# MIT-SPARK/Hydra-GNN

Measured on AMD Instinct MI355X. Metric: scene-graphs/sec (fwd+bwd) MP3D hetero batch, higher is better.
Workload: dtype f32

## Files before the change

### hydra-gnn_amd/csrc/aggregate.hip

```cpp
#include <type_traits>

#include "tail_fns.h"

namespace hmp {

KT_DEFINE(agg)
KT_BLOCKS_DEFINE(agg)

__device__ __forceinline__ int cdiv_dev(int a, int b) { return (a + b - 1) / b; }

__device__ __forceinline__ __amdgpu_buffer_rsrc_t buf_rsrc(const void* base, unsigned bytes) {
  return __builtin_amdgcn_make_buffer_rsrc(const_cast<void*>(base), 0, bytes, 0x00020000);
}

template <int VEC>
struct Acc;
template <>
struct Acc<4> {
  float4 v;
  __device__ __forceinline__ void zero() { v = make_float4(0.f, 0.f, 0.f, 0.f); }
  __device__ __forceinline__ void load(const float* p) { v = *reinterpret_cast<const float4*>(p); }
  __device__ __forceinline__ void store(float* p) const { *reinterpret_cast<float4*>(p) = v; }
  __device__ __forceinline__ void add(const Acc& o) { v.x += o.v.x; v.y += o.v.y; v.z += o.v.z; v.w += o.v.w; }
  __device__ __forceinline__ void add_div(const Acc& o, float d) {
// ... 519 lines not shown
    if (oi >= S.n_out) break;
    const TAggOut& O = S.out[oi];
    Acc<VEC> acc[NV];
#pragma unroll
    for (int q = 0; q < NV; ++q) acc[q].zero();
    gather_sum<GS, NV, VEC, GB>(acc, O.g, O.ldg, O.t_col, rb[oi], re[oi], c0, O.F, MeanW{O.rowptr, O.degf, a.mean});
#pragma unroll
    for (int q = 0; q < NV; ++q) {
      const int c = c0 + q * GS * VEC;
      if (c < O.F) put(acc[q], O.coff, c);
    }
  }
  }
  if (S.groot) {
#pragma unroll
    for (int q = 0; q < NV; ++q) {
      const int c = c0 + q * GS * VEC;
      if (c < S.Froot) {
        Acc<VEC> v;
        v.zero();
        if (live) load_z<GB>(v, S.groot, (int64_t)row * S.ldgr + c);
        put(v, S.roff, c);
      }
    }
  }
}

template <int GS, int NV, bool GB = false, bool DZB = false>
__global__ __launch_bounds__(256) void agg_bwd_kernel(const TAggArgs a) {
  if ((int)blockIdx.x == a.total_blocks) {
    finalize_loss(a.fin_row_lv, a.fin_rows, a.fin_out2, a.fin_state);
    return;
  }
  int si = 0;
  while (si + 1 < a.n && (int)blockIdx.x >= a.bstart[si + 1]) ++si;
  karg_warm<10>((int)offsetof(TAggArgs, s) + si * (int)sizeof(TAggSrc), (int)sizeof(TAggSrc));
  const TAggSrc& S = a.s[si];
  const int rpb = (S.tile_rows == 8 && 256 / GS > 8) ? 8 : 256 / GS;
  int local = blockIdx.x - S.block_start;
  if (a.xcd) local = (local & 7) * ((cdiv_dev(S.n_rows, rpb) + 7) >> 3) + (local >> 3);
  if ((int)threadIdx.x / GS >= rpb) return;
  int row = local * rpb + threadIdx.x / GS;
  if (GS == 64) row = __builtin_amdgcn_readfirstlane(row);
  if (row >= S.n_rows) return;
  agg_bwd_row<GS, NV, GB>(a, S, row, true, (int)(threadIdx.x % GS) * 4,
                          [&](Acc<4> v, int seg, int c) { store_z<DZB>(v, S.dz, (int64_t)row * S.lddz + seg + c); });
}

template <int GS>
__device__ __forceinline__ void agg_bwd_dx_tile(const TAggArgs& a, const TAggSrc& S, int row0, int row_end, float* Hs) {
  constexpr int TM = 16, LDH = 17, VEC = 4;
  constexpr int RPP = 256 / GS;
  constexpr int NP = TM / RPP;
  const int tid = threadIdx.x & 255;
  const int c0 = (tid % GS) * VEC;
  const int lane = threadIdx.x & 63, w = tid >> 6;
  const int nn = lane & 15, kq = lane >> 4;
  const int K = S.ncols;
  KT(8);
  constexpr int WB = 48;
#pragma unroll
  for (int p = 0; p < NP; ++p) {
    const int m = p * RPP + tid / GS;
    const int row = row0 + m;
    const bool live = row < row_end;
    agg_bwd_row<GS, 1, false>(a, S, row, live, c0, [&](Acc<VEC> v, int seg, int c) {
      if (live) v.store(S.dz + (int64_t)row * S.lddz + seg + c);
#pragma unroll
      for (int i = 0; i < 4; ++i) Hs[(seg + c + i) * LDH + m] = v.at(i);
    });
  }
  __syncthreads();
  if (S.xw == nullptr) return;
  KT(9);
  const int n_ct = (S.xN + 15) >> 4;
  for (int ct = w; ct < n_ct; ct += 4) {
    const int col = ct * 16 + nn;
    const float* wp = S.xw + min(col, S.xN - 1) + (int64_t)kq * S.xldw;
    const float* hp = Hs + kq * LDH + nn;
    f32x4 acc = {0.f, 0.f, 0.f, 0.f};
    float hv[4] = {0.f, 0.f, 0.f, 0.f};
    if (S.xh) {
#pragma unroll
      for (int r = 0; r < 4; ++r)
        hv[r] = S.xh[(int64_t)min(row0 + kq * 4 + r, row_end - 1) * S.xldh + min(col, S.xN - 1)];
    }
    for (int kb = 0; kb < K; kb += 4 * WB) {
      float bv[WB];
#pragma unroll
      for (int u = 0; u < WB; ++u) bv[u] = wp[(int64_t)min(kb + 4 * u, K - 4) * S.xldw];
#pragma unroll
      for (int u = 0; u < WB; ++u)
        if (kb + 4 * u < K) acc = __builtin_amdgcn_mfma_f32_16x16x4f32(hp[(kb + 4 * u) * LDH], bv[u], acc, 0, 0, 0);
    }
    if (col < S.xN) {
#pragma unroll
      for (int r = 0; r < 4; ++r) {
        const int row = row0 + kq * 4 + r;
        if (row >= row_end) continue;
        float v = acc[r];
        if (S.xh) {
          const float h = hv[r];
          const bool keep = !S.xdrop_on || (__float_as_uint(h) != 0x80000000u);
          float f = S.xscale;
          if (!keep) f = 0.f;
          else if (S.xact == HMP_ACT_RELU) f = h > 0.f ? S.xscale : 0.f;
          else if (S.xact == HMP_ACT_ELU) f = h > 0.f ? S.xscale : (h + S.xscale);
          v *= f;
        }
        S.xg[(int64_t)row * S.xldg + col] = v;
      }
    }
  }
  KT(10);
}

template <int GS>
__global__ __launch_bounds__(256) void agg_bwd_dx_kernel(const TAggArgs a) {
  extern __shared__ float Hs[];
  if ((int)blockIdx.x == a.total_blocks) {
    finalize_loss(a.fin_row_lv, a.fin_rows, a.fin_out2, a.fin_state);
    return;
  }
  KT_SPAN_BEGIN(48);
  int si = 0;
  while (si + 1 < a.n && (int)blockIdx.x >= a.bstart[si + 1]) ++si;
  karg_warm<10>((int)offsetof(TAggArgs, s) + si * (int)sizeof(TAggSrc), (int)sizeof(TAggSrc));
  const TAggSrc& S = a.s[si];
  const int row0 = ((int)blockIdx.x - S.block_start) * S.tile_rows;
  agg_bwd_dx_tile<GS>(a, S, row0, min(row0 + S.tile_rows, S.n_rows), Hs);
  KT_SPAN_END(48, si);
}

constexpr int WIN_THREADS = 1024;
constexpr int WIN_WAVES = WIN_THREADS / 64;
constexpr int WIN_ROW_BYTES = 512;
constexpr int WR = 64;
constexpr int WM = 64;
constexpr int WRING = 256;
constexpr int WG = WR / WIN_WAVES;
constexpr int WIDCAP = 3072;
constexpr int WRP = WR + 1;
constexpr int WIN_LDS_RING = (WRING + 1) * WIN_ROW_BYTES;
constexpr int WIN_LDS_IDS = 2 * WIDCAP * 4;
constexpr int WIN_LDS_RP = 3 * AGG_MAX_IN * WRP * 4;
constexpr int WIN_LDS_DEG = WRING * 4;
constexpr int WIN_LDS_FWD = WIN_LDS_RING + WIN_LDS_IDS + WIN_LDS_RP;
constexpr int WIN_LDS_BWD = WIN_LDS_FWD + WIN_LDS_DEG;
static_assert(WIN_LDS_BWD <= 160 * 1024, "LDS budget");
constexpr unsigned WIN_SKIP_OFF = 0xFFFFF000u;
typedef unsigned int u32x2 __attribute__((ext_vector_type(2)));

static_assert(AGG_MAX_IN == 6, "sel_q is written for 6 entries");
struct WinFwd {
  AggDst d;
  int mean;
  int n_chunks, chunks_per_block;
  int dbg;
};
struct WinBwd {
  TAggSrc s;
  int mean;
  int n_chunks, chunks_per_block;
};

// ... 642 lines not shown
    if (a.s[i].groot) Fmax = a.s[i].Froot > Fmax ? a.s[i].Froot : Fmax;
  }
  return Fmax;
}

int agg_bwd_launch(TAggArgs& a, hipStream_t st) {
  const int vec = 4;
  int Fmax = tagg_fmax(a);
  if (a.n == 0 || Fmax == 0) {
    if (!a.fin_row_lv) return HMP_OK;
    Fmax = 4;
  }
  int gs, nv;
  pick_shape(Fmax, vec, gs, nv);
  int64_t rows_total = 0;
  for (int i = 0; i < a.n; ++i) rows_total += a.s[i].n_rows;
  a.xcd = (rows_total >= AGG_XCD_ROWS && agg_xcd_enabled()) ? 1 : 0;
  for (int i = 0; i < a.n; ++i)
    if (a.xcd || a.gb16 || rows_total > 16 * AGG_SMALL_TILES) a.s[i].tile_rows = 0;
  int blocks = agg_layout_rows(a, gs);
  if (blocks == 0 && !a.fin_row_lv) return HMP_OK;
  if (a.gb16) {
    HMP_CHECK_ARG(gs == 64 && nv == 1, "agg_bwd: bf16 gradient rows need row widths in (128, 256], got %d", Fmax);
    if (agg_win_enabled()) {
      bool any;
      HMP_TRY(agg_win_peel(a, st, &any));
      if (any) {
        blocks = agg_layout_rows(a, gs);
        if (blocks == 0 && !a.fin_row_lv) return HMP_OK;
      }
    }
    const int grid = blocks + (a.fin_row_lv ? 1 : 0);
    sync_bstart(a);
    if (a.dzb16) hipLaunchKernelGGL((agg_bwd_kernel<64, 1, true, true>), dim3(grid), dim3(256), 0, st, a);
    else hipLaunchKernelGGL((agg_bwd_kernel<64, 1, true, false>), dim3(grid), dim3(256), 0, st, a);
    HMP_LAUNCH_CHECK();
    return HMP_OK;
  }
  HMP_CHECK_ARG(!a.dzb16, "agg_bwd: a bf16 dz needs bf16 gradient rows (the one-wavefront-per-row kernel)");
  const int grid = blocks + (a.fin_row_lv ? 1 : 0);
  sync_bstart(a);
#define LAUNCH_BWD(GS_, NV_) hipLaunchKernelGGL((agg_bwd_kernel<GS_, NV_>), dim3(grid), dim3(256), 0, st, a)
  HMP_DISPATCH_GS_NV(gs, nv, LAUNCH_BWD)
#undef LAUNCH_BWD
  HMP_LAUNCH_CHECK();
  return HMP_OK;
}

int agg_bwd_dx_launch(TAggArgs& a, hipStream_t st) {
  int Fmax = tagg_fmax(a), kmax = 0;
  for (int i = 0; i < a.n; ++i) {
    kmax = a.s[i].ncols > kmax ? a.s[i].ncols : kmax;
    HMP_CHECK_ARG((a.s[i].ncols & 3) == 0, "agg_bwd_dx: ncols must be padded to 4");
  }
  if (a.n == 0 || Fmax == 0) {
    if (!a.fin_row_lv) return HMP_OK;
    Fmax = 4;
  }
  HMP_CHECK_ARG(Fmax <= 256 && kmax <= 896, "agg_bwd_dx: segment width %d / stacked width %d not supported", Fmax, kmax);
  const int blocks = agg_layout_tiles(a);
  if (blocks == 0 && !a.fin_row_lv) return HMP_OK;
  const int grid = blocks + (a.fin_row_lv ? 1 : 0);
  const size_t smem = (size_t)kmax * 17 * sizeof(float);
  sync_bstart(a);
  switch (agg_tile_gs(Fmax)) {
    case 16: hipLaunchKernelGGL((agg_bwd_dx_kernel<16>), dim3(grid), dim3(256), smem, st, a); break;
    case 32: hipLaunchKernelGGL((agg_bwd_dx_kernel<32>), dim3(grid), dim3(256), smem, st, a); break;
    default: hipLaunchKernelGGL((agg_bwd_dx_kernel<64>), dim3(grid), dim3(256), smem, st, a); break;
  }
  HMP_LAUNCH_CHECK();
  return HMP_OK;
}

template <bool FWD>
static int segment_mean_dispatch(const float* in, int ldi, int F, const hmp_plan& plan, float* out, int ldo, hipStream_t st) {
  const bool vec_ok = ((ldi & 3) == 0) && ((ldo & 3) == 0) && ((reinterpret_cast<uintptr_t>(in) & 15) == 0) &&
                      ((reinterpret_cast<uintptr_t>(out) & 15) == 0) && ((F & 3) == 0);
  const int vec = vec_ok ? 4 : 1;
  const int Fmax = F;
  const int n_rows = FWD ? plan.n_dst : plan.n_src;
  if (n_rows == 0 || F == 0) return HMP_OK;
  int gs, nv;
  pick_shape(F, vec, gs, nv);
  const int blocks = cdiv(n_rows, 256 / gs);
#define LAUNCH_SM(GS_, NV_)                                                                                                   \
  do {                                                                                                                        \
    if (FWD) {                                                                                                                \
      if (vec_ok) hipLaunchKernelGGL((segment_mean_fwd_kernel<GS_, NV_, 4>), dim3(blocks), dim3(256), 0, st, in, ldi, F, plan.d_rowptr, plan.d_col, n_rows, out, ldo); \
      else hipLaunchKernelGGL((segment_mean_fwd_kernel<GS_, NV_, 1>), dim3(blocks), dim3(256), 0, st, in, ldi, F, plan.d_rowptr, plan.d_col, n_rows, out, ldo); \
    } else {                                                                                                                  \
      if (vec_ok) hipLaunchKernelGGL((segment_mean_bwd_kernel<GS_, NV_, 4>), dim3(blocks), dim3(256), 0, st, in, ldi, F, plan.d_t_rowptr, plan.d_t_col, plan.d_rowptr, n_rows, out, ldo); \
      else hipLaunchKernelGGL((segment_mean_bwd_kernel<GS_, NV_, 1>), dim3(blocks), dim3(256), 0, st, in, ldi, F, plan.d_t_rowptr, plan.d_t_col, plan.d_rowptr, n_rows, out, ldo); \
    }                                                                                                                         \
  } while (0)
  HMP_DISPATCH_GS_NV(gs, nv, LAUNCH_SM)
#undef LAUNCH_SM
  HMP_LAUNCH_CHECK();
  return HMP_OK;
}

}

extern "C" int hmp_segment_mean_fwd(const float* d_x, int32_t ldx, int32_t F, hmp_plan plan, float* d_out, int32_t ldo, void* stream) {
  using namespace hmp;
  HMP_CHECK_ARG(d_x && d_out && plan.d_rowptr, "hmp_segment_mean_fwd: null pointer");
  HMP_CHECK_ARG(F >= 0 && ldx >= F && ldo >= F, "hmp_segment_mean_fwd: bad widths");
  HMP_CHECK_ARG(plan.n_edges == 0 || plan.d_col, "hmp_segment_mean_fwd: null col");
  const int panel = ((ldx & 3) == 0 && (ldo & 3) == 0 && (F & 3) == 0) ? 1024 : 256;
  for (int c = 0; c < F; c += panel) {
    const int w = (F - c) < panel ? (F - c) : panel;
    HMP_TRY((segment_mean_dispatch<true>(d_x + c, ldx, w, plan, d_out + c, ldo, (hipStream_t)stream)));
  }
  return HMP_OK;
}

extern "C" int hmp_segment_mean_bwd(const float* d_gout, int32_t ldg, int32_t F, hmp_plan plan, float* d_gx, int32_t ldgx, void* stream) {
// ... 12 lines not shown
```

### hydra-gnn_amd/csrc/device_fns.h

```cpp
#pragma once
#include "kernels.h"

namespace hmp {

__device__ __forceinline__ int find_seg(const int64_t* __restrict__ off, int B, int64_t g) {
  int lo = 0, hi = B - 1;
  while (lo < hi) {
    const int mid = (lo + hi + 1) >> 1;
    if (off[mid] <= g) lo = mid; else hi = mid - 1;
  }
  return lo;
}


__device__ __forceinline__ void pack_item(const PackSeg& S, int item, const float* __restrict__ params, float* __restrict__ packed) {
  const int chunks = (S.ld_dst + 63) >> 6;
  const int r = item / chunks;
  if (r >= S.rows_pad) return;
  float* dst = packed + S.dst + (int64_t)r * S.ld_dst;
  const int c = (item % chunks) * 64 + (threadIdx.x & 63);
  if (c >= S.ld_dst) return;
  float v = 0.f;
  if (S.kind == PACK_SUM) {
    if (r < S.rows && c < S.cols)
      for (int q = 0; q < S.nsrc; ++q) v += params[S.src[q] + (int64_t)r * S.ld_src + c];
  } else if (S.kind == PACK_HEADS) {
    const int h = r / S.Cp, cc = r % S.Cp;
    if (h < S.H && cc < S.C && c < S.cols) v = params[S.src[0] + (int64_t)(h * S.C + cc) * S.ld_src + c];
  } else if (S.kind == PACK_ATTDOT) {
    if (r < S.H && c < S.cols) {
      const float* av = params + S.att + r * S.C;
      const float* wv = params + S.src[0] + (int64_t)(r * S.C) * S.ld_src + c;
      for (int cc = 0; cc < S.C; cc += 8) {
        float a8[8], w8[8];
#pragma unroll
        for (int u = 0; u < 8; ++u) {
          const int ci = min(cc + u, S.C - 1);
          a8[u] = av[ci];
          w8[u] = wv[(int64_t)ci * S.ld_src];
        }
#pragma unroll
        for (int u = 0; u < 8; ++u)
          if (cc + u < S.C) v += a8[u] * w8[u];
      }
    }
  } else {
    if (r < S.rows && c < S.H) {
      const float* av = params + S.att + c * S.C;
      const float* wv = params + S.src[0] + (int64_t)(c * S.C) * S.ld_src + r;
      for (int cc = 0; cc < S.C; cc += 8) {
        float a8[8], w8[8];
#pragma unroll
        for (int u = 0; u < 8; ++u) {
          const int ci = min(cc + u, S.C - 1);
          a8[u] = av[ci];
          w8[u] = wv[(int64_t)ci * S.ld_src];
        }
#pragma unroll
        for (int u = 0; u < 8; ++u)
          if (cc + u < S.C) v += a8[u] * w8[u];
      }
    }
  }
  dst[c] = v;
}

__device__ __forceinline__ void pack_block(const PackSeg* __restrict__ segs, const SegBlocks& sb, const float* __restrict__ params,
                                           float* __restrict__ packed, int* step_ctr, int* step_mirror, int blk) {
  if (step_ctr && blk == 0 && threadIdx.x == 0) {
    const int t = *step_ctr + 1;
    *step_ctr = t;
    if (step_mirror) *step_mirror = t;
  }
  int si = 0;
  while (si + 1 < sb.n && blk >= sb.start[si + 1]) ++si;
  const PackSeg S = segs[si];
  pack_item(S, (blk - sb.start[si]) * 4 + (int)(threadIdx.x >> 6), params, packed);
}

}
```

### hydra-gnn_amd/csrc/kernels.h

```cpp
#pragma once
#include "common.h"

namespace hmp {

enum { EPI_NONE = 0, EPI_ACTMASK = 1 };

struct GemmProblem {
  const float* A;
  const float* B;
  float* C;
  const float* H;
  int c_bf16;
  int a_bf16;
  int b_bf16;
  int h_bf16;
  const float* A2;
  int lda2, a_split;
  int64_t slab_stride;
  int M, N, K;
  int lda, ldb, ldc, ldh;
  int trans_a;
  int trans_b;
  int n_real;
  int aug_ones;
// ... 209 lines not shown
  int ldzr, roff;
  const float* bias;
  int n_in;
  int act;
  int drop_on;
  DropCfg drop;
  int block_start;
  const float* pw;
  float* pz;
  int pldw, pldz, pncols, pK;
  const int64_t* ce_labels;
  int64_t ce_ignored;
  int ce_classes, ce_ldg;
  float* ce_grad;
  float* ce_row_lv;
  const uint8_t* ce_mask;
  int ce_tail;
  int win_in;
  int tile_rows;
  AggIn in[AGG_MAX_IN];
};
struct AggArgs {
  int n;
  int total_blocks;
  int mean;
  int xcd;
  int zb16;
  int hb16;
  NetState* state;
  int bstart[HMP_MAX_NODE_TYPES];
  AggDst d[HMP_MAX_NODE_TYPES];
};
int agg_fwd_launch(AggArgs& a, hipStream_t st);
int agg_proj_fwd_launch(AggArgs& a, hipStream_t st);

struct TAggOut {
  const int* t_rowptr;
  const int* t_col;
  const int* rowptr;
  const float* degf;
  const float* g;
  int ldg, coff, F;
  int same_type;
  int n_dst;
};
struct TAggSrc {
  int n_rows;
  float* dz;
  int lddz, ncols;
  const float* groot;
  int ldgr, roff, Froot;
  int n_out;
  int block_start;
  const float* xw;
  float* xg;
  const float* xh;
  int xldw, xN, xldg, xldh, xact, xdrop_on;
  float xscale;
  int win_out;
  int tile_rows;
  TAggOut out[AGG_MAX_IN];
};
struct TAggArgs {
  int n;
  int total_blocks;
  int mean;
  int xcd;
  int gb16;
  int dzb16;
  const float* fin_row_lv;
  int fin_rows;
  float* fin_out2;
  NetState* fin_state;
  int bstart[HMP_MAX_NODE_TYPES];
  TAggSrc s[HMP_MAX_NODE_TYPES];
};
int agg_bwd_launch(TAggArgs& a, hipStream_t st);
int agg_bwd_dx_launch(TAggArgs& a, hipStream_t st);

int seg_mean_rows_launch(const void* x, int ldx, int x_bf16, int F, const int* rowptr, const int* col, int n_rows, float* m, int ldm,
                         hipStream_t st);
int seg_mean_rows_t_launch(const float* dm, int lddm, int F, const int* t_rowptr, const int* t_col, const float* degf, int n_rows,
                           const void* h, int ldh, int h_bf16, int act, int drop_on, float dscale, void* g, int ldg, int g_bf16, hipStream_t st);

enum { PACK_SUM = 0, PACK_HEADS = 1, PACK_ATTDOT = 2, PACK_ATTDOT_T = 3 };
struct PackSeg {
  int64_t dst;
  int rows, rows_pad, cols, ld_dst;
  int ld_src;
  int nsrc;
  int kind, H, C, Cp;
  int64_t att;
  int64_t src[AGG_MAX_IN];
};
constexpr int SEG_MAX = 400;
struct SegBlocks {
  int n;
  int start[SEG_MAX + 1];
};
int pack_launch(const PackSeg* d_segs, const SegBlocks& sb, const float* d_params, float* d_packed, int* step_ctr, int* step_mirror,
                hipStream_t st);

enum { GT_COPY = 0, GT_ATT_OUTER = 1, GT_ATT_DOT = 2, GT_ATT_OUTER_T = 3, GT_ATT_DOT_T = 4 };
struct GradTerm {
  int kind;
  int slab_id;
  int64_t src;
  int ld;
  int C, Cp;
  int inner;
  int64_t att, w;
  int ldw;
  float scale;
};
struct GradSeg {
  int64_t dst;
  int rows, cols;
  int n_terms;
  GradTerm t[3];
};
constexpr int SLAB_IDS_PER_LAYER = 2 * HMP_MAX_NODE_TYPES + HMP_MAX_CONVS;
constexpr int GRAD_MAX_SLAB_IDS = HMP_MAX_LAYERS * SLAB_IDS_PER_LAYER;
constexpr int HEAD_SLAB_ID = GRAD_MAX_SLAB_IDS;
struct GradReduceDyn {
  unsigned char n_slabs[GRAD_MAX_SLAB_IDS + 1];
  int slab_stride[GRAD_MAX_SLAB_IDS + 1];
};

constexpr int GAT_HMAX = 8;
constexpr int GAT_MAX_EDIM = 4;
constexpr int GAT_CMAX = 512;
constexpr int GAT_WIDE_HMAX = 4;
inline bool gat_shape_ok(int heads, int channels) {
  return heads >= 1 && heads <= GAT_HMAX && channels >= 1 && channels <= GAT_CMAX && (channels <= 256 || heads <= GAT_WIDE_HMAX);
}

struct GatInS {
  int et, src_t;
  const int *rowptr, *col, *eid, *t_rowptr, *t_col, *t_pos;
  const float* z;
  int ldz, hoff;
  const float* za;
  int ldza, asoff;
  const float* zd;
  int ldzd, adoff;
  const float* vedge;
  int edim;
// ... 153 lines not shown
```

### hydra-gnn_amd/csrc/net.hip

```cpp
#include <cstdlib>
#include <vector>

#include "plan_small.h"

using namespace hmp;

namespace {

struct ConvLayout {
  int coff;
  int asoff, adoff;
  int H, C, Cp;
  int64_t vedge_off;
  int64_t vslab_off;
  bool wd_is_src;
  float *smax, *sden, *alpha_drop, *dlogit, *dlogit_orig;
  bool agg_first;
  int aoff, ld_m;
  int64_t wc_off, cslab_off;
  float *mrows, *dmrows;
};

struct LayerLayout {
  int kind;
  int n_live;
  int live[HMP_MAX_CONVS];
  ConvLayout conv[HMP_MAX_CONVS];
  int n_in[HMP_MAX_NODE_TYPES];
  bool reads[HMP_MAX_NODE_TYPES];
  int aggf_of_src[HMP_MAX_NODE_TYPES];
  int ncols[HMP_MAX_NODE_TYPES];
  int roff[HMP_MAX_NODE_TYPES];
  int64_t wp_off[HMP_MAX_NODE_TYPES];
  int ldw[HMP_MAX_NODE_TYPES];
  int64_t bias_off[HMP_MAX_NODE_TYPES];
  int64_t slab_off[HMP_MAX_NODE_TYPES];
  int lddw[HMP_MAX_NODE_TYPES];
  int64_t bslab_off[HMP_MAX_NODE_TYPES];
  GatLayerS* d_gat;
  GatLayerS h_gat;
};

constexpr int MAX_SLABS = 192;
static_assert(MAX_SLABS >= GEMM_TALL_SLABS, "the slab buffer must hold what the tall weight-gradient kernel may write");
constexpr int TN_DIRECT_SLABS = 16;

struct ProfRec {
  int cls;
  hipEvent_t a, b;
};

}

struct EnvSwitches {
  bool plan_sliced = true;
  bool front = true;
  bool z16 = true;
  bool h16 = true;
  bool rootcopy = false;
  bool tn_direct = true;
  bool bf16_all = false;
};

struct StepCall {
  int training = 0;
  uint64_t seed = 0;
  uint32_t rng_step = 0;
  int* d_step = nullptr;
  const int64_t* ce_labels = nullptr;
  const hmp_head_targets* tgt = nullptr;
  int64_t ce_ignored = 0;
  AdamFuse adam = {};
  bool fin_loss = false;
  int fin_rows = 0;
  bool aux_g_ready = false;
  int head_blocks = 0;
  bool ce_done = false;
  bool tail_done[2] = {false, false};
  bool adam_done = false;
};

struct hmp_net {
  hmp_net_spec spec;
  EnvSwitches env;
  int T, ET, L;
  int dim[HMP_MAX_LAYERS + 1][HMP_MAX_NODE_TYPES];
  int ld[HMP_MAX_LAYERS + 1][HMP_MAX_NODE_TYPES];
// ... 159 lines not shown
      Y.reads[C.src] = Y.reads[C.dst] = true;
      if (Y.kind == HMP_CONV_SAGE) {
        HMP_CHECK_ARG(C.w0 >= 0 && C.b0 >= 0 && C.w1 >= 0, "net: SAGE conv needs lin_l.weight, lin_l.bias, lin_r.weight");
        if (aggf) {
          HMP_CHECK_ARG(Y.aggf_of_src[C.src] < 0, "net: layer %d has two aggregate-first convs from node type %d (at most one)", l, C.src);
          Y.aggf_of_src[C.src] = c;
          Q.agg_first = true;
          Q.ld_m = fpad(n->dim[l][C.src]);
          n->any_agg_first = true;
        } else {
          Q.coff = Y.ncols[C.src];
          Y.ncols[C.src] += fpad(C.f_out);
        }
      } else {
        HMP_CHECK_ARG(C.w0 >= 0 && C.a0 >= 0 && C.a1 >= 0 && C.b0 >= 0, "net: GAT conv needs lin_src, att_src, att_dst, bias");
        HMP_CHECK_ARG(C.edge_dim == 0 || (C.w2 >= 0 && C.a2 >= 0), "net: GAT_edge conv needs lin_edge, att_edge");
        Q.H = C.heads; Q.C = C.f_out; Q.Cp = fpad(C.f_out);
        Q.wd_is_src = (C.src == C.dst) || (C.w1 == C.w0) || (C.w1 < 0);
        HMP_CHECK_ARG(Q.wd_is_src ? (n->dim[l][C.src] == n->dim[l][C.dst]) : true, "net: shared lin with different widths");
        Q.coff = Y.ncols[C.src];
        Y.ncols[C.src] += Q.H * Q.Cp;
        Q.asoff = Y.ncols[C.src];
        Y.ncols[C.src] += fpad(Q.H);
        n->any_gat = true;
      }
    }
    HMP_CHECK_ARG(Y.n_live > 0, "net: layer %d has no live conv", l);
    if (Y.kind == HMP_CONV_SAGE) {
      for (int i = 0; i < Y.n_live; ++i) {
        const int c = Y.live[i];
        const hmp_conv_spec& C = Ls.convs[c];
        if (!Y.conv[c].agg_first) continue;
        Y.conv[c].aoff = Y.ncols[C.dst];
        Y.ncols[C.dst] += fpad(C.f_out);
      }
      for (int t = 0; t < n->T; ++t)
        if (Y.n_in[t] > 0) {
          Y.roff[t] = Y.ncols[t];
          Y.ncols[t] += fpad(Ls.out_dim[t]);
        }
    } else {
      for (int i = 0; i < Y.n_live; ++i) {
        const int c = Y.live[i];
        const hmp_conv_spec& C = Ls.convs[c];
        Y.conv[c].adoff = Y.ncols[C.dst];
        Y.ncols[C.dst] += fpad(C.heads);
      }
    }
    for (int t = 0; t < n->T; ++t) {
      Y.ldw[t] = fpad(n->dim[l][t]);
      Y.lddw[t] = fpad(n->dim[l][t] + 1);
      Y.wp_off[t] = packed;
      packed += (int64_t)Y.ncols[t] * Y.ldw[t];
      Y.bias_off[t] = packed;
      packed += (Y.n_in[t] > 0) ? fpad(Ls.out_dim[t]) : 0;
      Y.slab_off[t] = slabs;
      slabs += (int64_t)MAX_SLABS * Y.ncols[t] * Y.lddw[t];
      Y.bslab_off[t] = slabs;
      if (Y.kind == HMP_CONV_GAT && Y.n_in[t] > 0) slabs += (int64_t)MAX_SLABS * fpad(Ls.out_dim[t]) * 4;
    }
    for (int i = 0; i < Y.n_live; ++i) {
      const int c = Y.live[i];
      if (!Y.conv[c].agg_first) continue;
      const hmp_conv_spec& C = Ls.convs[c];
      Y.conv[c].wc_off = packed;
      packed += (int64_t)fpad(C.f_out) * Y.ldw[C.src];
      Y.conv[c].cslab_off = slabs;
      slabs += (int64_t)MAX_SLABS * fpad(C.f_out) * Y.lddw[C.src];
    }
    if (Y.kind == HMP_CONV_GAT) {
      for (int i = 0; i < Y.n_live; ++i) {
        const int c = Y.live[i];
        if (Ls.convs[c].edge_dim > 0) {
          Y.conv[c].vedge_off = packed;
          packed += GAT_MAX_EDIM * GAT_HMAX;
          Y.conv[c].vslab_off = slabs;
          slabs += (int64_t)MAX_SLABS * GAT_MAX_EDIM * GAT_HMAX;
        }
      }
    }
  }
  for (int l = 0; l < n->L; ++l) {
    const LayerLayout& Y = n->lay[l];
    for (int i = 0; i < Y.n_live; ++i) {
      const hmp_conv_spec& C = S.layers[l].convs[Y.live[i]];
      if (l == n->L - 1)
        HMP_CHECK_ARG(C.dst == S.readout_type || C.dst == S.aux_readout_type,
                      "net: last-layer conv %d is active but does not feed a readout type", Y.live[i]);
      else
        HMP_CHECK_ARG(n->lay[l + 1].reads[C.dst], "net: layer %d conv %d is active but layer %d never reads its output", l, Y.live[i], l + 1);
    }
  }
  n->packed_floats = packed;
  n->slab_floats = slabs;
  n->out_dim = n->dim[n->L][S.readout_type];
  n->out_ld = fpad(n->out_dim);
  HMP_CHECK_ARG(n->out_dim > 0, "net: readout type has no output in the last layer");
  HMP_CHECK_ARG(S.aux_readout_type < 0 || n->dim[n->L][S.aux_readout_type] > 0, "net: second readout type has no output in the last layer");
  return HMP_OK;
}

inline int slab_id_w(int l, int t) { return l * SLAB_IDS_PER_LAYER + t; }
inline int slab_id_b(int l, int t) { return l * SLAB_IDS_PER_LAYER + HMP_MAX_NODE_TYPES + t; }
inline int slab_id_v(int l, int c) { return l * SLAB_IDS_PER_LAYER + 2 * HMP_MAX_NODE_TYPES + c; }

GradTerm term(int kind, int slab_id, int64_t src, int ld, int C, int Cp, int inner = 0, int64_t att = 0, int64_t w = 0, int ldw = 0,
              float scale = 1.f) {
  GradTerm t;
  memset(&t, 0, sizeof(t));
  t.kind = kind; t.slab_id = slab_id; t.src = src; t.ld = ld; t.C = C; t.Cp = Cp; t.inner = inner;
  t.att = att; t.w = w; t.ldw = ldw; t.scale = scale;
  return t;
}

int build_tables(hmp_net* n) {
  const hmp_net_spec& S = n->spec;
  std::vector<PackSeg> ps;
  std::vector<int64_t> prs;
  std::vector<GradSeg> gs;
  std::vector<int64_t> ges;
  int64_t prow = 0, gel = 0;
  auto push_pack = [&](const PackSeg& s) {
    ps.push_back(s); prs.push_back(prow); prow += s.rows_pad;
    if (s.rows_pad > n->max_pack_rows) n->max_pack_rows = s.rows_pad;
  };
  auto push_grad = [&](GradSeg g) {
    gs.push_back(g); ges.push_back(gel); gel += (int64_t)g.rows * g.cols;
    if ((int64_t)g.rows * g.cols > n->max_grad_elems) n->max_grad_elems = (int64_t)g.rows * g.cols;
  };
  for (int l = 0; l < n->L; ++l) {
    const hmp_layer_spec& Ls = S.layers[l];
    const LayerLayout& Y = n->lay[l];
    const float gscale = Ls.group_mean ? 1.f : 1.f;
    (void)gscale;
    for (int i = 0; i < Y.n_live; ++i) {
      const int c = Y.live[i];
      const hmp_conv_spec& C = Ls.convs[c];
      const ConvLayout& Q = Y.conv[c];
      const int fs = n->dim[l][C.src], ft = n->dim[l][C.dst];
      PackSeg s;
      memset(&s, 0, sizeof(s));
      if (Y.kind == HMP_CONV_SAGE) {
        s.kind = PACK_SUM;
        s.dst = Q.agg_first ? Q.wc_off : Y.wp_off[C.src] + (int64_t)Q.coff * Y.ldw[C.src];
        s.rows = C.f_out; s.rows_pad = fpad(C.f_out); s.cols = fs; s.ld_dst = Y.ldw[C.src]; s.ld_src = fs;
        s.nsrc = 1; s.src[0] = C.w0;
        push_pack(s);
        GradSeg g;
        memset(&g, 0, sizeof(g));
        g.dst = C.w0; g.rows = C.f_out; g.cols = fs; g.n_terms = 1;
        if (Q.agg_first) g.t[0] = term(GT_COPY, slab_id_v(l, c), Q.cslab_off, Y.lddw[C.src], C.f_out, C.f_out);
        else g.t[0] = term(GT_COPY, slab_id_w(l, C.src), Y.slab_off[C.src] + (int64_t)Q.coff * Y.lddw[C.src], Y.lddw[C.src], C.f_out, C.f_out);
        push_grad(g);
        continue;
      }
      const int HC = Q.H * Q.C;
      const int64_t wd = Q.wd_is_src ? C.w0 : C.w1;
      s.kind = PACK_HEADS; s.H = Q.H; s.C = Q.C; s.Cp = Q.Cp;
      s.dst = Y.wp_off[C.src] + (int64_t)Q.coff * Y.ldw[C.src];
      s.rows = Q.H * Q.Cp; s.rows_pad = Q.H * Q.Cp; s.cols = fs; s.ld_dst = Y.ldw[C.src]; s.ld_src = fs;
      s.nsrc = 1; s.src[0] = C.w0;
      push_pack(s);
      s.kind = PACK_ATTDOT; s.dst = Y.wp_off[C.src] + (int64_t)Q.asoff * Y.ldw[C.src];
      s.rows = Q.H; s.rows_pad = fpad(Q.H); s.att = C.a0; s.src[0] = C.w0;
      push_pack(s);
      s.dst = Y.wp_off[C.dst] + (int64_t)Q.adoff * Y.ldw[C.dst];
      s.cols = ft; s.ld_dst = Y.ldw[C.dst]; s.ld_src = ft; s.att = C.a1; s.src[0] = wd;
      push_pack(s);
      if (C.edge_dim > 0) {
        s.kind = PACK_ATTDOT_T; s.dst = Q.vedge_off; s.rows = C.edge_dim; s.rows_pad = GAT_MAX_EDIM; s.cols = Q.H;
        s.ld_dst = GAT_HMAX; s.ld_src = C.edge_dim; s.att = C.a2; s.src[0] = C.w2;
        push_pack(s);
      }
      const int64_t S_hs = Y.slab_off[C.src] + (int64_t)Q.coff * Y.lddw[C.src];
      const int64_t S_as = Y.slab_off[C.src] + (int64_t)Q.asoff * Y.lddw[C.src];
      const int64_t S_ad = Y.slab_off[C.dst] + (int64_t)Q.adoff * Y.lddw[C.dst];
      GradSeg g;
      memset(&g, 0, sizeof(g));
      g.dst = C.w0; g.rows = HC; g.cols = fs;
      g.t[g.n_terms++] = term(GT_COPY, slab_id_w(l, C.src), S_hs, Y.lddw[C.src], Q.C, Q.Cp);
      g.t[g.n_terms++] = term(GT_ATT_OUTER, slab_id_w(l, C.src), S_as, Y.lddw[C.src], Q.C, Q.C, 0, C.a0);
      if (Q.wd_is_src) g.t[g.n_terms++] = term(GT_ATT_OUTER, slab_id_w(l, C.dst), S_ad, Y.lddw[C.dst], Q.C, Q.C, 0, C.a1);
      push_grad(g);
      if (!Q.wd_is_src) {
        memset(&g, 0, sizeof(g));
        g.dst = C.w1; g.rows = HC; g.cols = ft; g.n_terms = 1;
        g.t[0] = term(GT_ATT_OUTER, slab_id_w(l, C.dst), S_ad, Y.lddw[C.dst], Q.C, Q.C, 0, C.a1);
        push_grad(g);
      }
      memset(&g, 0, sizeof(g));
      g.dst = C.a0; g.rows = HC; g.cols = 1; g.n_terms = 1;
      g.t[0] = term(GT_ATT_DOT, slab_id_w(l, C.src), S_as, Y.lddw[C.src], Q.C, Q.C, fs, 0, C.w0, fs);
      push_grad(g);
      memset(&g, 0, sizeof(g));
      g.dst = C.a1; g.rows = HC; g.cols = 1; g.n_terms = 1;
      g.t[0] = term(GT_ATT_DOT, slab_id_w(l, C.dst), S_ad, Y.lddw[C.dst], Q.C, Q.C, ft, 0, wd, ft);
      push_grad(g);
      if (C.edge_dim > 0) {
        memset(&g, 0, sizeof(g));
        g.dst = C.w2; g.rows = HC; g.cols = C.edge_dim; g.n_terms = 1;
        g.t[0] = term(GT_ATT_OUTER_T, slab_id_v(l, c), Q.vslab_off, GAT_HMAX, Q.C, Q.C, 0, C.a2);
        push_grad(g);
        memset(&g, 0, sizeof(g));
        g.dst = C.a2; g.rows = HC; g.cols = 1; g.n_terms = 1;
        g.t[0] = term(GT_ATT_DOT_T, slab_id_v(l, c), Q.vslab_off, GAT_HMAX, Q.C, Q.C, C.edge_dim, 0, C.w2, C.edge_dim);
        push_grad(g);
      }
      memset(&g, 0, sizeof(g));
      const int wout = Ls.out_dim[C.dst];
      g.dst = C.b0; g.rows = wout; g.cols = 1; g.n_terms = 1;
      g.t[0] = term(GT_COPY, slab_id_b(l, C.dst), Y.bslab_off[C.dst], 4, wout, wout, 0, 0, 0, 0,
                    Ls.group_mean ? 1.f / (float)Y.n_in[C.dst] : 1.f);
      push_grad(g);
    }
    for (int t = 0; t < n->T; ++t) {
      if (Y.n_in[t] == 0) continue;
      const int fo = Ls.out_dim[t], ft = n->dim[l][t];
      PackSeg s, b;
      memset(&s, 0, sizeof(s));
      memset(&b, 0, sizeof(b));
      s.kind = PACK_SUM; b.kind = PACK_SUM;
      s.dst = Y.wp_off[t] + (int64_t)(Y.roff[t] < 0 ? 0 : Y.roff[t]) * Y.ldw[t];
      s.rows = fo; s.rows_pad = fpad(fo); s.cols = ft; s.ld_dst = Y.ldw[t]; s.ld_src = ft;
      b.dst = Y.bias_off[t];
      b.rows = 1; b.rows_pad = 1; b.cols = fo; b.ld_dst = fpad(fo); b.ld_src = fo;
      for (int i = 0; i < Y.n_live; ++i) {
        const hmp_conv_spec& C = Ls.convs[Y.live[i]];
        if (C.dst != t) continue;
        b.src[b.nsrc++] = C.b0;
        if (Y.kind != HMP_CONV_SAGE) continue;
        s.src[s.nsrc++] = C.w1;
        GradSeg g;
        memset(&g, 0, sizeof(g));
        g.dst = C.w1; g.rows = fo; g.cols = ft; g.n_terms = 1;
        const int64_t root = Y.slab_off[t] + (int64_t)Y.roff[t] * Y.lddw[t];
        g.t[0] = term(GT_COPY, slab_id_w(l, t), root, Y.lddw[t], fo, fo);
        push_grad(g);
        memset(&g, 0, sizeof(g));
        g.dst = C.b0; g.rows = fo; g.cols = 1; g.n_terms = 1;
        g.t[0] = term(GT_COPY, slab_id_w(l, t), root + ft, Y.lddw[t], fo, fo);
        push_grad(g);
      }
      if (Y.kind == HMP_CONV_SAGE) push_pack(s);
      push_pack(b);
    }
  }
  prs.push_back(prow);
  ges.push_back(gel);
  n->n_pack = (int)ps.size(); n->pack_rows = prow;
  n->n_grad = (int)gs.size(); n->grad_elems = gel;
  HMP_CHECK_ARG(ps.size() <= (size_t)SEG_MAX && gs.size() <= (size_t)SEG_MAX, "net: too many parameter segments (%zu / %zu > %d)",
                ps.size(), gs.size(), SEG_MAX);
  n->pack_sb.n = (int)ps.size();
  n->pack_sb.start[0] = 0;
  for (size_t i = 0; i < ps.size(); ++i)
    n->pack_sb.start[i + 1] = n->pack_sb.start[i] + cdiv((int64_t)ps[i].rows_pad * cdiv(ps[i].ld_dst, 64), 4);
  {
    std::vector<int2> pm;
    for (size_t i = 0; i < ps.size(); ++i) {
      const int items = ps[i].rows_pad * cdiv(ps[i].ld_dst, 64);
      for (int it = 0; it < items; it += 16) pm.push_back(make_int2((int)i, it));
    }
    n->n_pack_blocks16 = (int)pm.size();
    if (!pm.empty()) {
      HMP_HIP(hipMalloc(&n->d_pack_map, pm.size() * sizeof(int2)));
      HMP_HIP(hipMemcpy(n->d_pack_map, pm.data(), pm.size() * sizeof(int2), hipMemcpyHostToDevice));
    }
  }
  n->grad_sb.n = (int)gs.size();
  n->grad_sb.start[0] = 0;
  for (size_t i = 0; i < gs.size(); ++i) {
    const bool wave_mode = gs[i].n_terms == 1 && (gs[i].t[0].kind == GT_ATT_DOT || gs[i].t[0].kind == GT_ATT_DOT_T);
    const int64_t el = (int64_t)gs[i].rows * gs[i].cols;
    n->grad_sb.start[i + 1] = n->grad_sb.start[i] + cdiv(el, wave_mode ? 4 : 256);
  }
  HMP_HIP(hipMalloc(&n->d_pack_segs, ps.size() * sizeof(PackSeg)));
  HMP_HIP(hipMalloc(&n->d_grad_segs, gs.size() * sizeof(GradSeg)));
  HMP_HIP(hipMemcpy(n->d_pack_segs, ps.data(), ps.size() * sizeof(PackSeg), hipMemcpyHostToDevice));
  HMP_HIP(hipMemcpy(n->d_grad_segs, gs.data(), gs.size() * sizeof(GradSeg), hipMemcpyHostToDevice));
  for (int l = 0; l < n->L; ++l)
    if (n->lay[l].kind == HMP_CONV_GAT) HMP_HIP(hipMalloc(&n->lay[l].d_gat, sizeof(GatLayerS)));
  return HMP_OK;
}

size_t carve(hmp_net* n, char* base, const int32_t* cn, const int64_t* ce) {
  size_t off = 0;
  n->sadd_floats = 0;
  auto take = [&](size_t bytes) -> char* {
    char* p = base ? base + off : nullptr;
    off += align256(bytes);
    return p;
  };
  const hmp_net_spec& S = n->spec;
  for (int e = 0; e < n->ET; ++e) {
    const int ns = cn[S.edge_src[e]], nd = cn[S.edge_dst[e]];
    hmp_plan& P = n->plan[e];
// ... 670 lines not shown
        n->call.fin_loss = false;
        fin_early = true;
      }
      for (int s = 0; s < n->T; ++s) {
        if (Y.ncols[s] == 0 || b->n_nodes[s] == 0) continue;
        TAggSrc& T = a.s[a.n++];
        T.n_rows = b->n_nodes[s];
        T.dz = n->dZ[l][s]; T.lddz = Y.ncols[s]; T.ncols = Y.ncols[s];
        if (Y.roff[s] >= 0) {
          int ldg;
          T.groot = g_of(s, ldg);
          T.ldgr = ldg; T.roff = Y.roff[s]; T.Froot = fpad(Ls.out_dim[s]);
        }
        for (int i = 0; i < Y.n_live; ++i) {
          const int c = Y.live[i];
          const hmp_conv_spec& C = Ls.convs[c];
          if (Y.conv[c].agg_first) {
            if (C.dst != s || b->n_nodes[C.src] == 0 || b->n_edges[C.edge_type] == 0) continue;
            TAggOut& O = T.out[T.n_out++];
            O.t_rowptr = n->d_iota; O.t_col = n->d_iota; O.rowptr = n->d_iota; O.degf = n->d_ones;
            int ldg;
            O.g = g_of(s, ldg);
            O.ldg = ldg; O.coff = Y.conv[c].aoff; O.F = fpad(C.f_out);
            O.same_type = 0; O.n_dst = b->n_nodes[s];
            continue;
          }
          if (C.src != s) continue;
          TAggOut& O = T.out[T.n_out++];
          const hmp_plan& P = n->plan[C.edge_type];
          O.t_rowptr = P.d_t_rowptr; O.t_col = P.d_t_col; O.rowptr = P.d_rowptr; O.degf = n->degf[C.edge_type];
          int ldg;
          O.g = g_of(C.dst, ldg);
          O.ldg = ldg; O.coff = Y.conv[c].coff; O.F = fpad(C.f_out);
          O.same_type = C.src == C.dst ? 1 : 0;
          O.n_dst = b->n_nodes[C.dst];
          if (n->fuse_now && b->n_edges[C.edge_type] > (int64_t)8 * b->n_nodes[C.src]) T.tile_rows = 8;
        }
      }
      dx_fused = n->fuse_now && l > 0;
      int fmax = 0;
      for (int i = 0; i < a.n && dx_fused; ++i) {
        if (a.s[i].ncols > 896) dx_fused = false;
        for (int o = 0; o < a.s[i].n_out; ++o) fmax = a.s[i].out[o].F > fmax ? a.s[i].out[o].F : fmax;
        if (a.s[i].groot) fmax = a.s[i].Froot > fmax ? a.s[i].Froot : fmax;
      }
      if (fmax > 256) dx_fused = false;
      if (dx_fused) {
        const hmp_layer_spec& Lp = S.layers[l - 1];
        int ai = 0;
        for (int s = 0; s < n->T; ++s) {
          if (Y.ncols[s] == 0 || b->n_nodes[s] == 0) continue;
          TAggSrc& T = a.s[ai++];
          if (!n->G[l][s]) continue;
          T.xw = n->d_packed + Y.wp_off[s]; T.xldw = Y.ldw[s]; T.xN = n->dim[l][s];
          T.xg = n->G[l][s]; T.xldg = n->ld[l][s];
          T.xdrop_on = (n->training && Lp.dropout > 0.f) ? 1 : 0;
          T.xact = Lp.act;
          T.xscale = T.xdrop_on ? 1.f / (1.f - Lp.dropout) : 1.f;
          T.xh = (T.xact != HMP_ACT_NONE || T.xdrop_on) ? n->H[l][s] : nullptr;
          T.xldh = n->ld[l][s];
        }
        HMP_TRY(agg_bwd_dx_launch(a, st));
      } else {
        a.gb16 = g16[l + 1] ? 1 : 0;
        dz16 = a.gb16 && n->compute_bf16 != 0;
        for (int s = 0; s < n->T && dz16; ++s)
          if (Y.ncols[s] > 0 && b->n_nodes[s] > 0 && (Y.ncols[s] % 256) != 0) dz16 = false;
        if (!n->env.z16) dz16 = false;
        a.dzb16 = dz16 ? 1 : 0;
        rootless = dz16;
        for (int i = 0; i < a.n && rootless; ++i)
          if (a.s[i].groot && ((a.s[i].roff & 255) != 0 || a.s[i].Froot != 256 || (a.s[i].ldgr & 3) != 0)) rootless = false;
        if (n->env.rootcopy) rootless = false;
        if (rootless)
          for (int i = 0; i < a.n; ++i) a.s[i].groot = nullptr;
        HMP_TRY(agg_bwd_launch(a, st));
      }
    }
    const bool need_dx = !dx_fused && ((l > 0) || (d_gx != nullptr));
    auto dz_at = [&](int t, int col) -> const float* {
      return dz16 ? reinterpret_cast<const float*>(reinterpret_cast<const uint16_t*>(n->dZ[l][t]) + col) : n->dZ[l][t] + col;
    };
    auto aggf_live = [&](int c) {
      const hmp_conv_spec& C = Ls.convs[c];
      return Y.conv[c].agg_first && b->n_nodes[C.dst] > 0 && b->n_nodes[C.src] > 0 && b->n_edges[C.edge_type] > 0;
    };
    if (need_dx && n->any_agg_first) {
      std::vector<GemmProblem> pp;
      for (int i = 0; i < Y.n_live; ++i) {
        const int c = Y.live[i];
        if (!aggf_live(c)) continue;
        const hmp_conv_spec& C = Ls.convs[c];
        float* want = l > 0 ? n->G[l][C.src] : d_gx[C.src];
        if (!want) continue;
        const ConvLayout& Q = Y.conv[c];
        GemmProblem p;
        memset(&p, 0, sizeof(p));
        p.A = dz_at(C.dst, Q.aoff); p.lda = Y.ncols[C.dst]; p.trans_a = 0; p.a_bf16 = dz16 ? 1 : 0;
        p.B = n->d_packed + Q.wc_off; p.ldb = Y.ldw[C.src]; p.trans_b = 0;
        p.C = Q.dmrows; p.ldc = Q.ld_m;
        p.M = b->n_nodes[C.dst]; p.N = n->dim[l][C.src]; p.K = fpad(C.f_out);
        p.n_real = p.N;
        p.epi = EPI_NONE;
        pp.push_back(p);
      }
      if (!pp.empty()) {
        Scope sp(n, KC_GEMM_BWD, st);
// ... 801 lines not shown
```

Measured before the change: 371,700.

## Use a transposed, swizzled weight image for vectorized loads in the fused dx GEMM

The parameter packer now also writes a transposed copy of each SAGE layer's weights, with padding and a column swizzle, so the fused input-gradient tile can fetch four K values per lane with one float4 load. Before, it issued one strided scalar load per MFMA step. For the GS=16 variant, the first column tile's weights and activations are prefetched before the barrier so their latency overlaps the aggregation phase. The cost is extra packed-parameter memory, extra packing writes every step, a larger padded shared-memory tile, and higher register pressure from the prefetch buffer.

```diff
diff --git a/hydra-gnn_amd/csrc/aggregate.hip b/hydra-gnn_amd/csrc/aggregate.hip
--- a/hydra-gnn_amd/csrc/aggregate.hip
+++ b/hydra-gnn_amd/csrc/aggregate.hip
@@ -595,13 +595,28 @@
   constexpr int TM = 16, LDH = 17, VEC = 4;
   constexpr int RPP = 256 / GS;
   constexpr int NP = TM / RPP;
+  constexpr int WB = 12;
   const int tid = threadIdx.x & 255;
   const int c0 = (tid % GS) * VEC;
   const int lane = threadIdx.x & 63, w = tid >> 6;
   const int nn = lane & 15, kq = lane >> 4;
-  const int K = S.ncols;
+  const int K = S.ncols, K16 = (K + 15) & ~15;
   KT(8);
-  constexpr int WB = 48;
+  constexpr bool EARLY = GS == 16;
+  const int n_ct = S.xwt ? (S.xN + 15) >> 4 : 0;
+  float4 pre[WB];
+  auto fetch_first = [&]() {
+    if (w >= n_ct) return;
+    const float* wrow = S.xwt + (int64_t)min(w * 16 + nn, S.xN - 1) * S.xldt + 4 * kq;
+#pragma unroll
+    for (int i = 0; i < WB; ++i) pre[i] = *reinterpret_cast<const float4*>(wrow + min(16 * i, K16 - 16));
+  };
+  float hv0[4] = {0.f, 0.f, 0.f, 0.f};
+  if (EARLY && S.xh && w < n_ct) {
+#pragma unroll
+    for (int r = 0; r < 4; ++r)
+      hv0[r] = S.xh[(int64_t)min(row0 + kq * 4 + r, row_end - 1) * S.xldh + min(w * 16 + nn, S.xN - 1)];
+  }
 #pragma unroll
   for (int p = 0; p < NP; ++p) {
     const int m = p * RPP + tid / GS;
@@ -613,28 +628,46 @@
       for (int i = 0; i < 4; ++i) Hs[(seg + c + i) * LDH + m] = v.at(i);
     });
   }
+  if constexpr (EARLY) fetch_first();
+  for (int i = tid; i < (K16 - K) * TM; i += 256) Hs[(K + (i >> 4)) * LDH + (i & 15)] = 0.f;
   __syncthreads();
-  if (S.xw == nullptr) return;
+  if (S.xwt == nullptr) return;
   KT(9);
-  const int n_ct = (S.xN + 15) >> 4;
-  for (int ct = w; ct < n_ct; ct += 4) {
+  auto trip = [&](int kb, const float4 (&bv)[WB], f32x4& acc) {
+#pragma unroll
+    for (int i = 0; i < WB; ++i) {
+      const int k = kb + 16 * i;
+      if (k >= K) break;
+      const float* hp = Hs + (k + kq) * LDH + nn;
+      acc = __builtin_amdgcn_mfma_f32_16x16x4f32(hp[0 * LDH], bv[i].x, acc, 0, 0, 0);
+      acc = __builtin_amdgcn_mfma_f32_16x16x4f32(hp[4 * LDH], bv[i].y, acc, 0, 0, 0);
+      acc = __builtin_amdgcn_mfma_f32_16x16x4f32(hp[8 * LDH], bv[i].z, acc, 0, 0, 0);
+      acc = __builtin_amdgcn_mfma_f32_16x16x4f32(hp[12 * LDH], bv[i].w, acc, 0, 0, 0);
+    }
+  };
+  auto tile = [&](int ct, auto first) {
     const int col = ct * 16 + nn;
-    const float* wp = S.xw + min(col, S.xN - 1) + (int64_t)kq * S.xldw;
-    const float* hp = Hs + kq * LDH + nn;
+    const float* wrow = S.xwt + (int64_t)min(col, S.xN - 1) * S.xldt + 4 * kq;
     f32x4 acc = {0.f, 0.f, 0.f, 0.f};
     float hv[4] = {0.f, 0.f, 0.f, 0.f};
-    if (S.xh) {
+    if constexpr (decltype(first)::value) {
+#pragma unroll
+      for (int r = 0; r < 4; ++r) hv[r] = hv0[r];
+    } else if (S.xh) {
 #pragma unroll
       for (int r = 0; r < 4; ++r)
         hv[r] = S.xh[(int64_t)min(row0 + kq * 4 + r, row_end - 1) * S.xldh + min(col, S.xN - 1)];
     }
-    for (int kb = 0; kb < K; kb += 4 * WB) {
-      float bv[WB];
-#pragma unroll
-      for (int u = 0; u < WB; ++u) bv[u] = wp[(int64_t)min(kb + 4 * u, K - 4) * S.xldw];
-#pragma unroll
-      for (int u = 0; u < WB; ++u)
-        if (kb + 4 * u < K) acc = __builtin_amdgcn_mfma_f32_16x16x4f32(hp[(kb + 4 * u) * LDH], bv[u], acc, 0, 0, 0);
+    int kb = 0;
+    if constexpr (decltype(first)::value) {
+      trip(0, pre, acc);
+      kb = 16 * WB;
+    }
+    for (; kb < K; kb += 16 * WB) {
+      float4 bv[WB];
+#pragma unroll
+      for (int i = 0; i < WB; ++i) bv[i] = *reinterpret_cast<const float4*>(wrow + min(kb + 16 * i, K16 - 16));
+      trip(kb, bv, acc);
     }
     if (col < S.xN) {
 #pragma unroll
@@ -654,6 +687,12 @@
         S.xg[(int64_t)row * S.xldg + col] = v;
       }
     }
+  };
+  if constexpr (EARLY) {
+    if (w < n_ct) tile(w, std::true_type());
+    for (int ct = w + 4; ct < n_ct; ct += 4) tile(ct, std::false_type());
+  } else {
+    for (int ct = w; ct < n_ct; ct += 4) tile(ct, std::false_type());
   }
   KT(10);
 }
@@ -1402,6 +1441,8 @@
   for (int i = 0; i < a.n; ++i) {
     kmax = a.s[i].ncols > kmax ? a.s[i].ncols : kmax;
     HMP_CHECK_ARG((a.s[i].ncols & 3) == 0, "agg_bwd_dx: ncols must be padded to 4");
+    HMP_CHECK_ARG(!a.s[i].xwt || (a.s[i].xldt == ((a.s[i].ncols + 15) & ~15) && a.s[i].xN > 0),
+                  "agg_bwd_dx: transposed weights of %d columns with leading dimension %d", a.s[i].ncols, a.s[i].xldt);
   }
   if (a.n == 0 || Fmax == 0) {
     if (!a.fin_row_lv) return HMP_OK;
@@ -1411,7 +1452,7 @@
   const int blocks = agg_layout_tiles(a);
   if (blocks == 0 && !a.fin_row_lv) return HMP_OK;
   const int grid = blocks + (a.fin_row_lv ? 1 : 0);
-  const size_t smem = (size_t)kmax * 17 * sizeof(float);
+  const size_t smem = (size_t)((kmax + 15) & ~15) * 17 * sizeof(float);
   sync_bstart(a);
   switch (agg_tile_gs(Fmax)) {
     case 16: hipLaunchKernelGGL((agg_bwd_dx_kernel<16>), dim3(grid), dim3(256), smem, st, a); break;
diff --git a/hydra-gnn_amd/csrc/device_fns.h b/hydra-gnn_amd/csrc/device_fns.h
--- a/hydra-gnn_amd/csrc/device_fns.h
+++ b/hydra-gnn_amd/csrc/device_fns.h
@@ -13,12 +13,13 @@
 }
 
 
-__device__ __forceinline__ void pack_item(const PackSeg& S, int item, const float* __restrict__ params, float* __restrict__ packed) {
+__host__ __device__ __forceinline__ void pack_lane(const PackSeg& S, int item, int lane, const float* __restrict__ params,
+                                                   float* __restrict__ packed) {
   const int chunks = (S.ld_dst + 63) >> 6;
   const int r = item / chunks;
   if (r >= S.rows_pad) return;
   float* dst = packed + S.dst + (int64_t)r * S.ld_dst;
-  const int c = (item % chunks) * 64 + (threadIdx.x & 63);
+  const int c = (item % chunks) * 64 + lane;
   if (c >= S.ld_dst) return;
   float v = 0.f;
   if (S.kind == PACK_SUM) {
@@ -63,6 +64,15 @@
     }
   }
   dst[c] = v;
+  if (S.ld_dst_t > 0) {
+    float* dt = packed + S.dst_t + (int64_t)c * S.ld_dst_t;
+    dt[wpt_col(S.col_t + r)] = v;
+    for (int p = r; p < S.pad_t; p += S.rows_pad) dt[wpt_col(S.col_t + S.rows_pad + p)] = 0.f;
+  }
+}
+
+__device__ __forceinline__ void pack_item(const PackSeg& S, int item, const float* __restrict__ params, float* __restrict__ packed) {
+  pack_lane(S, item, (int)(threadIdx.x & 63), params, packed);
 }
 
 __device__ __forceinline__ void pack_block(const PackSeg* __restrict__ segs, const SegBlocks& sb, const float* __restrict__ params,
diff --git a/hydra-gnn_amd/csrc/kernels.h b/hydra-gnn_amd/csrc/kernels.h
--- a/hydra-gnn_amd/csrc/kernels.h
+++ b/hydra-gnn_amd/csrc/kernels.h
@@ -285,10 +285,10 @@
   int ldgr, roff, Froot;
   int n_out;
   int block_start;
-  const float* xw;
+  const float* xwt;
   float* xg;
   const float* xh;
-  int xldw, xN, xldg, xldh, xact, xdrop_on;
+  int xldt, xN, xldg, xldh, xact, xdrop_on;
   float xscale;
   int win_out;
   int tile_rows;
@@ -325,7 +325,10 @@
   int kind, H, C, Cp;
   int64_t att;
   int64_t src[AGG_MAX_IN];
-};
+  int64_t dst_t;
+  int ld_dst_t, col_t, pad_t;
+};
+__host__ __device__ inline int wpt_col(int k) { return (k & ~15) | ((k & 3) << 2) | ((k >> 2) & 3); }
 constexpr int SEG_MAX = 400;
 struct SegBlocks {
   int n;
diff --git a/hydra-gnn_amd/csrc/net.hip b/hydra-gnn_amd/csrc/net.hip
--- a/hydra-gnn_amd/csrc/net.hip
+++ b/hydra-gnn_amd/csrc/net.hip
@@ -33,6 +33,8 @@
   int roff[HMP_MAX_NODE_TYPES];
   int64_t wp_off[HMP_MAX_NODE_TYPES];
   int ldw[HMP_MAX_NODE_TYPES];
+  int64_t wpt_off[HMP_MAX_NODE_TYPES];
+  int ldt[HMP_MAX_NODE_TYPES];
   int64_t bias_off[HMP_MAX_NODE_TYPES];
   int64_t slab_off[HMP_MAX_NODE_TYPES];
   int lddw[HMP_MAX_NODE_TYPES];
@@ -298,6 +300,9 @@
       Y.lddw[t] = fpad(n->dim[l][t] + 1);
       Y.wp_off[t] = packed;
       packed += (int64_t)Y.ncols[t] * Y.ldw[t];
+      Y.wpt_off[t] = packed;
+      Y.ldt[t] = (l >= 1 && Y.kind == HMP_CONV_SAGE && Y.ncols[t] > 0) ? ((Y.ncols[t] + 15) & ~15) : 0;
+      packed += (int64_t)Y.ldw[t] * Y.ldt[t];
       Y.bias_off[t] = packed;
       packed += (Y.n_in[t] > 0) ? fpad(Ls.out_dim[t]) : 0;
       Y.slab_off[t] = slabs;
@@ -366,6 +371,13 @@
   std::vector<GradSeg> gs;
   std::vector<int64_t> ges;
   int64_t prow = 0, gel = 0;
+  auto with_wpt = [&](PackSeg& s, const LayerLayout& Y, int t, int coff) {
+    if (Y.ldt[t] == 0) return;
+    s.dst_t = Y.wpt_off[t];
+    s.col_t = coff;
+    s.ld_dst_t = Y.ldt[t];
+    s.pad_t = coff + s.rows_pad == Y.ncols[t] ? Y.ldt[t] - Y.ncols[t] : 0;
+  };
   auto push_pack = [&](const PackSeg& s) {
     ps.push_back(s); prs.push_back(prow); prow += s.rows_pad;
     if (s.rows_pad > n->max_pack_rows) n->max_pack_rows = s.rows_pad;
@@ -391,6 +403,7 @@
         s.dst = Q.agg_first ? Q.wc_off : Y.wp_off[C.src] + (int64_t)Q.coff * Y.ldw[C.src];
         s.rows = C.f_out; s.rows_pad = fpad(C.f_out); s.cols = fs; s.ld_dst = Y.ldw[C.src]; s.ld_src = fs;
         s.nsrc = 1; s.src[0] = C.w0;
+        if (!Q.agg_first) with_wpt(s, Y, C.src, Q.coff);
         push_pack(s);
         GradSeg g;
         memset(&g, 0, sizeof(g));
@@ -487,7 +500,10 @@
         g.t[0] = term(GT_COPY, slab_id_w(l, t), root + ft, Y.lddw[t], fo, fo);
         push_grad(g);
       }
-      if (Y.kind == HMP_CONV_SAGE) push_pack(s);
+      if (Y.kind == HMP_CONV_SAGE) {
+        with_wpt(s, Y, t, Y.roff[t] < 0 ? 0 : Y.roff[t]);
+        push_pack(s);
+      }
       push_pack(b);
     }
   }
@@ -1264,7 +1280,8 @@
           if (Y.ncols[s] == 0 || b->n_nodes[s] == 0) continue;
           TAggSrc& T = a.s[ai++];
           if (!n->G[l][s]) continue;
-          T.xw = n->d_packed + Y.wp_off[s]; T.xldw = Y.ldw[s]; T.xN = n->dim[l][s];
+          HMP_CHECK_ARG(Y.ldt[s] > 0, "net: layer %d type %d has no transposed weight image for the fused input gradient", l, s);
+          T.xwt = n->d_packed + Y.wpt_off[s]; T.xldt = Y.ldt[s]; T.xN = n->dim[l][s];
           T.xg = n->G[l][s]; T.xldg = n->ld[l][s];
           T.xdrop_on = (n->training && Lp.dropout > 0.f) ? 1 : 0;
           T.xact = Lp.act;
```

Measured after the change: 376,200 (median of 6 runs). 1.2% higher.
